# acids-ircam/RAVE

Measured on NVIDIA H100. Metric: audio-seconds/s (v2 train step fwd+bwd, 48 kHz), higher is better.
Workload: dtype bf16

## Files before the change

include/rave_b200.h:

```cpp
#ifndef RAVE_B200_H
#define RAVE_B200_H

#include <stddef.h>
#include <stdint.h>

#ifdef __cplusplus
extern "C" {
#endif

#define RAVE_ACT_NONE 0
#define RAVE_ACT_LEAKY 1
#define RAVE_ACT_SNAKE 2

#define RAVE_PREC_FP32 0
#define RAVE_PREC_BF16 1
#define RAVE_PREC_TF32 2

int rave_b200_version(void);
const char *rave_b200_last_error(void);
unsigned long long rave_b200_launch_count(void);

int rave_pqmf_analysis_fwd(const float *x, const float *taps, float *y, int B, int T, int Lout,
                           int ntaps, int pad_l, int flip_sign, void *stream);
int rave_pqmf_synthesis_fwd(const float *x, const float *w, float *out, int B, int L, int K,
// ... 65 lines not shown
                           void *stream);
int rave_time_stack_nhwc(const float *x, void *out_bf16, int B, int C, int T, int F, long sb, long st, int Fp, int Cp, int kt,
                         int pt, void *stream);
int rave_time_stack_nhwc_bwd(const void *g_bf16, float *gx, int B, int C, int T, int F, int Fp, int Cp, int kt, int pt,
                             void *stream);
int rave_time_stack_nhwc_dil(const float *x, void *out_bf16, int B, int C, int T, int F, long sb, long st, int Fp, int Cp,
                             int kt, int pt, int dil, void *stream);
int rave_time_stack_nhwc_dil_bwd(const void *g_bf16, float *gx, int B, int C, int T, int F, int Fp, int Cp, int kt, int pt,
                                 int dil, void *stream);
int rave_l1_stats_f32(const float *t, const float *v, float *stats, long n, void *stream);
int rave_l1_grad_f32(const float *t, const float *v, const float *d, float *gt, float *gv, long n, void *stream);
int rave_leaky_fm_fwd(const float *x, float *a, float *stats, long H, float slope, void *stream);
int rave_leaky_fm_bwd(const float *a, const float *g, const float *d, float *gx, long H, float slope, void *stream);
int rave_leaky_fm_stack_fwd(const float *x, float *a, float *stats, void *xs_bf16, long Rh, int T, int F, int C, int Fp,
                            float slope, void *stream);
int rave_leaky_fm_stack_bwd(const float *a, const void *gxs_bf16, const float *ga, const float *d, float *gx, long Rh, int T,
                            int F, int C, int Fp, float slope, void *stream);
int rave_leaky_fm_stack_dil_fwd(const float *x, float *a, float *stats, void *xs_bf16, long Rh, int T, int F, int C, int Fp,
                                int dil, float slope, void *stream);
int rave_leaky_fm_stack_dil_bwd(const float *a, const void *gxs_bf16, const float *ga, const float *d, float *gx, long Rh,
                                int T, int F, int C, int Fp, int dil, float slope, void *stream);
int rave_snake_cl_fwd(const void *h_bf16, const float *alpha, void *a_bf16, long rows, int C, void *stream);
int rave_snake_cl_bwd(const void *ga_bf16, const void *h_bf16, const float *alpha, const void *add_bf16, void *gh_bf16,
                      float *dalpha, long rows, int C, void *stream);
int rave_conv1d_tc_wgrad(const void *P_bf16, const void *Q_bf16, float *dwt, float *dbias, int B, int Cm, int Lp,
                         int p_pitch, int Cn, int Lq, int q_pitch, int K, int stride, int dil, int pad_l,
                         void *stream);
int rave_tapmajor_to_weight_f32(const float *dwt, float *dw, int Cm, int Cn, int K, int transpose, int splits,
                                void *stream);
int rave_conv1d_c1_fwd(const float *x, const float *w, const float *bias, float *out_f32, void *out_act_bf16,
                       int R, int x_pitch, int Lin, int Cout, int Lout, int out_pitch, int K, int stride,
                       int pad_l, int act, float slope, void *stream);
int rave_conv1d_c1_wgrad_splits(int R, int Lout);
int rave_conv1d_c1_wgrad(const void *g_bf16, const float *x, float *dwt, int R, int x_pitch, int Lin, int Cout,
                         int Cg, int Lout, int g_pitch, int K, int stride, int pad_l, void *stream);
int rave_conv1d_c1_dgrad(const void *g_bf16, const float *w, float *dx, int R, int x_pitch, int Lin, int Cout,
                         int Cg, int Lout, int g_pitch, int K, int stride, int pad_l, void *stream);
int rave_colsum_bf16(const void *g_bf16, float *out, int R, int L, int pitch, int Cg, int C, void *stream);
int rave_im2col_c1(const float *src, void *X_bf16, int R, int src_pitch, int src_len, int Lin, int Lout,
                   int out_pitch, int K, int stride, int pad_l, int period, int pool, void *stream);
int rave_gather_c1(const float *P, float *dsrc, int R, int src_pitch, int src_len, int Lin, int Lout, int p_pitch,
                   int K, int stride, int pad_l, int period, int pool, void *stream);
int rave_im2col_cin(const float *src, void *X_bf16, int R, int cin, int src_pitch, int src_len, int Lin, int Lout,
                    int out_pitch, int W, int K, int stride, int pad_l, int period, int pool, void *stream);
int rave_gather_cin(const float *P, float *dsrc, int R, int cin, int src_pitch, int src_len, int Lin, int Lout,
                    int p_pitch, int W, int K, int stride, int pad_l, int period, int pool, void *stream);
int rave_fm_stats(const void *a_bf16, float *stats, int Bh, int L, int pitch, int C, float slope, void *stream);
int rave_fm_grad(const void *a_bf16, const float *dstats, void *gout_bf16, int Bh, int L, int pitch, int C,
                 float slope, void *stream);
int rave_score_stats(const float *score, float *stats, int Bh, int L, int pitch, int C, void *stream);
int rave_score_grad(const float *score, const float *dstats, void *gout_bf16, int Bh, int L, int pitch, int C,
                    void *stream);

int rave_spectral_stats(const void *X_c64, const void *Y_c64, float *stats, long n, float eps, void *stream);
int rave_spectral_grad(const void *X_c64, const void *Y_c64, void *dY_c64, const float *stats, const float *gup,
                       long n, float eps, void *stream);
int rave_stft_frames(const float *x, const float *window, float *frames, int N, int T, int n_fft, int hop,
                     void *stream);
int rave_stft_frames_bwd(const float *dframes, const float *window, float *dx, int N, int T, int n_fft, int hop,
                         void *stream);
int rave_stft_frames_valid(const float *x, const float *window, float *frames, int N, int T, int n_fft, int hop,
                           float scale, void *stream);
int rave_stft_frames_valid_bwd(const float *dframes, const float *window, float *dx, int N, int T, int n_fft, int hop,
                               float scale, void *stream);
int rave_rfft_bwd_scale(const void *G_c64, void *Z_c64, long N, int F, int bins, long sN, long sF, long sB,
                        void *stream);

int rave_weight_prep_tc(const float *v, const float *g, float *norm, void *outA_bf16, const int *tapsA, int nA,
                        void *outB_bf16, const int *tapsB, int nB, int C0, int C1, int K, int C0p, int C1p,
                        void *stream);
int rave_weight_norm_bwd_tapmajor(const float *dwt, const float *v, const float *g, const float *norm, float *dv,
                                  float *dg, int C0, int C1, int K, int C0p, int C1p, int splits, void *stream);
typedef struct rave_wprep_layer {
  const float *v, *g;
  float *norm;
  void *outA, *outB;
  const float *dwt;
  float *dv, *dg;
  int C0, C1, K, C0p, C1p, nA, nB, splits;
  int tapsA[32], tapsB[32];
} rave_wprep_layer;
int rave_weight_prep_tc_multi(int n, const rave_wprep_layer *layers, void *stream);
int rave_weight_prep_tc_multi_x3(int n, const rave_wprep_layer *layers, void *stream);
int rave_weight_norm_bwd_multi(int n, const rave_wprep_layer *layers, void *stream);
int rave_ncl_to_cl(const float *x, void *y_bf16, float *y_f32, int B, int C, int L, int act, float slope,
                   const float *alpha, void *stream);
int rave_cl_to_ncl(const float *x_cl, float *y, int B, int C, int L, void *stream);
int rave_ncl_to_cl_x3(const float *x, void *y_bf16, int B, int C, int L, void *stream);
int rave_act_to_bf16(const float *x, void *y_bf16, int B, int C, int L, int act, float slope,
                     const float *alpha, void *stream);
int rave_weight_to_tapmajor_bf16(const float *w, void *wt_bf16, int Cout, int Cin, int K, int transpose,
                                 int flip, void *stream);

int rave_noise_fir_fwd(const float *h, const float *M, const float *noise, float *out, int B, int C, int NB, int T,
                       int TS, void *stream);
int rave_noise_fir_bwd(const float *h, const float *M, const float *noise, const float *dout, float *dh, int B, int C,
                       int NB, int T, int TS, void *stream);

int rave_mel_log1p_fwd(const void *X_c64, const int *band, const float *weights, float *out, int N, int F, int bins,
                       int M, int nnz, float scale, void *stream);
int rave_mel_log1p_bwd(const void *X_c64, const int *band, const float *weights, const float *dy, void *dX_c64, int N,
                       int F, int bins, int M, int nnz, float scale, void *stream);

int rave_gru_fwd(const float *gi, const float *w_hh, const float *b_hh, float *h_out, float *save, int B, int T, int H,
                 void *stream);
int rave_gru_bwd(const float *dy, const float *save, const float *w_hh, float *dgi, float *dgh, int B, int T, int H,
                 void *stream);
int rave_gemm_f32_splits(int M, int N, int K);
int rave_gemm_f32(const float *A, long sam, long sak, const float *B, long sbk, long sbn, const float *bias, float *C,
// ... 25 lines not shown
```

rave_b200/_lib.py:

```python
import ctypes
import os
from ctypes import c_float, c_int, c_long, c_size_t, c_ulonglong, c_void_p, c_char_p

_HERE = os.path.dirname(os.path.abspath(__file__))
LIB_PATH = os.path.join(_HERE, "csrc", "librave_b200.so")

_P, _I, _F, _L = c_void_p, c_int, c_float, c_long

SIGNATURES = {
    "rave_b200_version": (c_int, []),
    "rave_b200_last_error": (c_char_p, []),
    "rave_b200_launch_count": (c_ulonglong, []),
    "rave_pqmf_analysis_fwd": (c_int, [_P, _P, _P, _I, _I, _I, _I, _I, _I, _P]),
    "rave_pqmf_synthesis_fwd": (c_int, [_P, _P, _P, _I, _I, _I, _I, _F, _I, _P]),
    "rave_pqmf_analysis_fast": (c_int, [_P, _P, _P, _P, _I, _I, _I, _I, _I, _P]),
    "rave_pqmf_synthesis_fast": (c_int, [_P, _P, _P, _P, _I, _I, _I, _F, _I, _P]),
    "rave_conv1d_gather_f32": (c_int, [_P, _P, _P, _P, _P, _I, _I, _I, _I, _I, _I, _I, _I, _I, _L, _L,
                                       _I, _F, _P, _I, _F, _P, _P, _P]),
    "rave_conv1d_scatter_f32": (c_int, [_P, _P, _P, _P, _P, _I, _I, _I, _I, _I, _I, _I, _I, _I, _L, _L,
                                        _I, _F, _P, _I, _F, _P, _P, _P]),
    "rave_conv1d_wgrad_workspace_bytes": (c_size_t, [_I, _I, _I, _I, _I]),
    "rave_conv1d_wgrad_f32": (c_int, [_P, _P, _P, _I, _I, _I, _I, _I, _I, _I, _I, _I, _L, _L, _I, _I,
                                      _F, _P, _P, _P]),
    "rave_weight_norm_fwd": (c_int, [_P, _P, _P, _P, _I, _I, _P]),
# ... 5 lines not shown
    "rave_reparam_fwd": (c_int, [_P, _P, _P, _P, _I, _I, _I, _P]),
    "rave_mmd_fwd": (c_int, [_P, _P, _P, _P, _I, _I, _I, _P]),
    "rave_mmd_bwd": (c_int, [_P, _P, _P, _P, _I, _I, _I, _P]),
    "rave_sphere_norm_fwd": (c_int, [_P, _P, _P, _I, _I, _I, _P]),
    "rave_sphere_norm_bwd": (c_int, [_P, _P, _P, _P, _I, _I, _I, _P]),
    "rave_latent_moments": (c_int, [_P, _I, _I, _I, _I, _P, _P, _P]),
    "rave_latent_moments_workspace_bytes": (c_long, [_I, _I, _I]),
    "rave_conv1d_tc_supported": (c_int, [_I, _I, _I, _I, _I]),
    "rave_dilated_unit_tc_supported": (c_int, [_I, _I]),
    "rave_dilated_unit_tc_fwd": (c_int, [_P, _P, _P, _P, _P, _P, _I, _I, _I, _I, _I, _I, _F, _F, _I, _F, _P]),
    "rave_conv1d_tc_plan": (c_int, [_I, _I, _I, _I, _I]),
    "rave_conv1d_tc_pp_stages": (c_int, [_I, _I, _I, _I, _I, _I, _I]),
    "rave_conv1d_tc_pp_fwd_stages": (c_int, [_I, _I, _I, _I, _I]),
    "rave_conv1d_tc_fwd": (c_int, [_P, _P, _P, _P, _P, _P, _P, _F, _P, _P, _I, _I, _I, _I, _I, _I, _I, _I, _I, _I, _I,
                                   _F, _I, _I, _I, _P, _I, _P]),
    "rave_conv1d_tc_fwd_x3": (c_int, [_P, _P, _P, _P, _P, _F, _P, _P, _I, _I, _I, _I, _I, _I, _I, _I, _I, _I, _I, _F, _I,
                                      _I, _I, _I, _P]),
    "rave_weight_prep_tc_multi_x3": (c_int, [_I, _P, _P]),
    "rave_ncl_to_cl_x3": (c_int, [_P, _P, _I, _I, _I, _P]),
    "rave_conv1d_tc_wgrad": (c_int, [_P, _P, _P, _P, _I, _I, _I, _I, _I, _I, _I, _I, _I, _I, _I, _P]),
    "rave_tapmajor_to_weight_f32": (c_int, [_P, _P, _I, _I, _I, _I, _I, _P]),
    "rave_conv1d_tc_wgrad_splits": (c_int, [_I, _I, _I, _I, _I]),
    "rave_time_stack_cl": (c_int, [_P, _P, _I, _I, _I, _I, _I, _I, _I, _I, _P]),
    "rave_time_stack_cl_bwd": (c_int, [_P, _P, _I, _I, _I, _I, _I, _I, _I, _I, _P]),
    "rave_time_stack_nhwc": (c_int, [_P, _P, _I, _I, _I, _I, ctypes.c_long, ctypes.c_long, _I, _I, _I, _I, _P]),
    "rave_time_stack_nhwc_bwd": (c_int, [_P, _P, _I, _I, _I, _I, _I, _I, _I, _I, _P]),
    "rave_time_stack_nhwc_dil": (c_int, [_P, _P, _I, _I, _I, _I, ctypes.c_long, ctypes.c_long, _I, _I, _I, _I, _I, _P]),
    "rave_time_stack_nhwc_dil_bwd": (c_int, [_P, _P, _I, _I, _I, _I, _I, _I, _I, _I, _I, _P]),
    "rave_l1_stats_f32": (c_int, [_P, _P, _P, ctypes.c_long, _P]),
    "rave_leaky_fm_fwd": (c_int, [_P, _P, _P, ctypes.c_long, ctypes.c_float, _P]),
    "rave_leaky_fm_bwd": (c_int, [_P, _P, _P, _P, ctypes.c_long, ctypes.c_float, _P]),
    "rave_leaky_fm_stack_fwd": (c_int, [_P, _P, _P, _P, ctypes.c_long, _I, _I, _I, _I, ctypes.c_float, _P]),
    "rave_leaky_fm_stack_bwd": (c_int, [_P, _P, _P, _P, _P, ctypes.c_long, _I, _I, _I, _I, ctypes.c_float, _P]),
    "rave_leaky_fm_stack_dil_fwd": (c_int, [_P, _P, _P, _P, ctypes.c_long, _I, _I, _I, _I, _I, ctypes.c_float, _P]),
    "rave_leaky_fm_stack_dil_bwd": (c_int, [_P, _P, _P, _P, _P, ctypes.c_long, _I, _I, _I, _I, _I, ctypes.c_float, _P]),
    "rave_l1_grad_f32": (c_int, [_P, _P, _P, _P, _P, ctypes.c_long, _P]),
    "rave_snake_cl_fwd": (c_int, [_P, _P, _P, ctypes.c_long, _I, _P]),
    "rave_snake_cl_bwd": (c_int, [_P, _P, _P, _P, _P, _P, ctypes.c_long, _I, _P]),
    "rave_weight_prep_tc": (c_int, [_P, _P, _P, _P, _P, _I, _P, _P, _I, _I, _I, _I, _I, _I, _P]),
    "rave_weight_norm_bwd_tapmajor": (c_int, [_P, _P, _P, _P, _P, _P, _I, _I, _I, _I, _I, _I, _P]),
    "rave_conv1d_c1_fwd": (c_int, [_P, _P, _P, _P, _P, _I, _I, _I, _I, _I, _I, _I, _I, _I, _I, _F, _P]),
    "rave_conv1d_c1_wgrad_splits": (c_int, [_I, _I]),
    "rave_conv1d_c1_wgrad": (c_int, [_P, _P, _P, _I, _I, _I, _I, _I, _I, _I, _I, _I, _I, _P]),
    "rave_conv1d_c1_dgrad": (c_int, [_P, _P, _P, _I, _I, _I, _I, _I, _I, _I, _I, _I, _I, _P]),
    "rave_colsum_bf16": (c_int, [_P, _P, _I, _I, _I, _I, _I, _P]),
    "rave_im2col_c1": (c_int, [_P, _P, _I, _I, _I, _I, _I, _I, _I, _I, _I, _I, _I, _P]),
    "rave_gather_c1": (c_int, [_P, _P, _I, _I, _I, _I, _I, _I, _I, _I, _I, _I, _I, _P]),
    "rave_im2col_cin": (c_int, [_P, _P, _I, _I, _I, _I, _I, _I, _I, _I, _I, _I, _I, _I, _I, _P]),
    "rave_gather_cin": (c_int, [_P, _P, _I, _I, _I, _I, _I, _I, _I, _I, _I, _I, _I, _I, _I, _P]),
    "rave_fm_stats": (c_int, [_P, _P, _I, _I, _I, _I, _F, _P]),
    "rave_fm_grad": (c_int, [_P, _P, _P, _I, _I, _I, _I, _F, _P]),
    "rave_score_stats": (c_int, [_P, _P, _I, _I, _I, _I, _P]),
    "rave_score_grad": (c_int, [_P, _P, _P, _I, _I, _I, _I, _P]),
    "rave_spectral_stats": (c_int, [_P, _P, _P, _L, _F, _P]),
    "rave_spectral_grad": (c_int, [_P, _P, _P, _P, _P, _L, _F, _P]),
    "rave_stft_frames": (c_int, [_P, _P, _P, _I, _I, _I, _I, _P]),
    "rave_stft_frames_bwd": (c_int, [_P, _P, _P, _I, _I, _I, _I, _P]),
    "rave_stft_frames_valid": (c_int, [_P, _P, _P, _I, _I, _I, _I, _F, _P]),
    "rave_stft_frames_valid_bwd": (c_int, [_P, _P, _P, _I, _I, _I, _I, _F, _P]),
    "rave_rfft_bwd_scale": (c_int, [_P, _P, _L, _I, _I, _L, _L, _L, _P]),
    "rave_mel_log1p_fwd": (c_int, [_P, _P, _P, _P, _I, _I, _I, _I, _I, _F, _P]),
    "rave_mel_log1p_bwd": (c_int, [_P, _P, _P, _P, _P, _I, _I, _I, _I, _I, _F, _P]),
    "rave_gru_fwd": (c_int, [_P, _P, _P, _P, _P, _I, _I, _I, _P]),
    "rave_gru_bwd": (c_int, [_P, _P, _P, _P, _P, _I, _I, _I, _P]),
    "rave_gemm_f32_splits": (c_int, [_I, _I, _I]),
    "rave_gemm_f32": (c_int, [_P, _L, _L, _P, _L, _L, _P, _P, _L, _P, _I, _I, _I, _P, _I, _P]),
    "rave_noise_fir_fwd": (c_int, [_P, _P, _P, _P, _I, _I, _I, _I, _I, _P]),
    "rave_noise_fir_bwd": (c_int, [_P, _P, _P, _P, _P, _I, _I, _I, _I, _I, _P]),
    "rave_adam_multi": (c_int, [_I, _P, _P, _P, _P, _P, _P, _P, _F, _F, _F, _P]),
    "rave_weight_prep_tc_multi": (c_int, [_I, _P, _P]),
    "rave_weight_norm_bwd_multi": (c_int, [_I, _P, _P]),
    "rave_ncl_to_cl": (c_int, [_P, _P, _P, _I, _I, _I, _I, _F, _P, _P]),
    "rave_cl_to_ncl": (c_int, [_P, _P, _I, _I, _I, _P]),
    "rave_act_to_bf16": (c_int, [_P, _P, _I, _I, _I, _I, _F, _P, _P]),
    "rave_weight_to_tapmajor_bf16": (c_int, [_P, _P, _I, _I, _I, _I, _I, _P]),
    "rave_prior_latent_classes": (c_int, [_P, _P, _P, _P, _P, _I, _I, _I, _I, _I, _P]),
    "rave_prior_embed_fwd": (c_int, [_P, _P, _P, _P, _P, _I, _I, _I, _I, _I, _I, _I, _F, _P]),
    "rave_prior_embed_wgrad": (c_int, [_P, _P, _P, _P, _P, _I, _I, _I, _I, _I, _I, _I, _F, _P]),
    "rave_gate_fwd": (c_int, [_P, _P, _I, _I, _I, _I, _P]),
    "rave_gate_bwd": (c_int, [_P, _P, _P, _I, _I, _I, _I, _P]),
    "rave_prior_head_ce_fwd": (c_int, [_P, _P, _P, _P, _P, _I, _I, _I, _I, _I, _I, _F, _P]),
    "rave_prior_head_ce_bwd": (c_int, [_P, _P, _P, _P, _P, _P, _P, _P, _I, _I, _I, _I, _I, _I, _F, _P]),
}



class WPrepLayer(ctypes.Structure):
    _fields_ = [("v", c_void_p), ("g", c_void_p), ("norm", c_void_p), ("outA", c_void_p), ("outB", c_void_p),
                ("dwt", c_void_p), ("dv", c_void_p), ("dg", c_void_p),
                ("C0", c_int), ("C1", c_int), ("K", c_int), ("C0p", c_int), ("C1p", c_int), ("nA", c_int),
                ("nB", c_int), ("splits", c_int), ("tapsA", c_int * 32), ("tapsB", c_int * 32)]


_lib = None


class RaveB200Error(RuntimeError):
    pass


def load():
    global _lib
    if _lib is not None:
        return _lib
    if not os.path.isfile(LIB_PATH):
        raise RaveB200Error(
            f"{LIB_PATH} not found: build it with `python -c 'import __graft_entry__ as g; g.build()'` "
            "(rave_b200 has no CPU or PyTorch fallback)")
# ... 55 lines not shown
```

rave_b200/core.py:

```python
from typing import Callable, Optional, Sequence

import numpy as np
import torch
import torch.nn as nn


def mod_sigmoid(x):
    return 2 * torch.sigmoid(x) ** 2.3 + 1e-7


def get_augmented_latent_size(latent_size: int, noise_augmentation: int):
    return latent_size + noise_augmentation


def hinge_gan(score_real, score_fake):
    loss_dis = (torch.relu(1 - score_real) + torch.relu(1 + score_fake)).mean()
    loss_gen = -score_fake.mean()
    return loss_dis, loss_gen


def ls_gan(score_real, score_fake):
    loss_dis = ((score_real - 1).pow(2) + score_fake.pow(2)).mean()
    loss_gen = (score_fake - 1).pow(2).mean()
    return loss_dis, loss_gen
# ... 154 lines not shown
        f = fb.detach().cpu()
        rows, wts, off = [], [], 0
        for m in range(f.shape[1]):
            nz = torch.nonzero(f[:, m]).reshape(-1)
            lo, hi = (int(nz[0]), int(nz[-1]) + 1) if nz.numel() else (0, 0)
            rows.append((lo, hi, off))
            wts.append(f[lo:hi, m])
            off += hi - lo
        w = torch.cat(wts) if off else torch.zeros(1)
        table = (torch.tensor(rows, dtype=torch.int32).to(fb.device), w.contiguous().to(fb.device))
        self.__dict__["_bands"] = (fb, fb._version, table)
        return table

    def encode_log1p(self, x: torch.Tensor) -> torch.Tensor:
        from . import ops
        batch, channels, T = x.shape
        w = self.spectrogram.window
        if x.requires_grad and torch.is_grad_enabled():
            X = ops.rfft(ops.stft_frames(x.reshape(-1, T), w, self.n_fft, self.hop_length), self._rfft_bw())
            band, wts = self.band_table()
            return ops.MelLog1pFn.apply(X, band, wts, self.n_mels, 1.0 / float(self._win_energy()), batch, channels)
        with torch.no_grad():
            frames = ops.stft_frames(x.detach().reshape(-1, T), w, self.n_fft, self.hop_length)
            X = torch.fft.rfft(frames)
            band, wts = self.band_table()
            return ops.mel_log1p(X, band, wts, self.n_mels, 1.0 / float(self._win_energy()), batch, channels)

    def _rfft_bw(self):
        w = self.spectrogram.window
        hit = self.__dict__.get("_rfft_bw_cache")
        if hit is None or hit.device != w.device:
            bw = torch.full((self.n_fft // 2 + 1,), 0.5 * self.n_fft)
            bw[0] = bw[-1] = self.n_fft
            hit = self.__dict__["_rfft_bw_cache"] = bw.to(w.device)
        return hit

    def _win_energy(self):
        w = self.spectrogram.window
        hit = self.__dict__.get("_energy")
        if hit is None or hit[0] is not w or hit[1] != w._version:
            hit = self.__dict__["_energy"] = (w, w._version, float(w.detach().double().square().sum().cpu()))
        return hit[2]


class AudioDistanceV1(nn.Module):

    def __init__(self, multiscale_stft: Callable[[], nn.Module], log_epsilon: float) -> None:
        super().__init__()
        self.multiscale_stft = multiscale_stft()
        self.log_epsilon = log_epsilon

    def forward(self, x, y):
        mstft = self.multiscale_stft
        if (x.is_cuda and not x.requires_grad and isinstance(mstft, MultiScaleSTFT) and mstft.magnitude
                and x.dtype == torch.float32):
            from . import ops
            distance = 0.
            for sx, sy in zip(mstft.complex_stfts(x), mstft.complex_stfts(y)):
                distance = distance + ops.spectral_distance(sx, sy, self.log_epsilon)
            return {"spectral_distance": distance}
        stfts_x = self.multiscale_stft(x)
        stfts_y = self.multiscale_stft(y)
        distance = 0.
        for sx, sy in zip(stfts_x, stfts_y):
            logx = torch.log(sx + self.log_epsilon)
            logy = torch.log(sy + self.log_epsilon)
            distance = distance + mean_difference(sx, sy, norm="L2", relative=True) \
                + mean_difference(logx, logy, norm="L1")
        return {"spectral_distance": distance}


def _is_recurrent(module) -> bool:
    return hasattr(module, "gru_state") or hasattr(module, "temporal")


@torch.enable_grad()
def get_rave_receptive_field(model, n_channels=1):
    from . import engine, pqmf
    N = 2 ** 15
    device = next(iter(model.parameters())).device
    was_training, precision = model.training, engine.precision()
    recurrent = [m for m in model.modules() if _is_recurrent(m)]
    banks = [m for m in model.modules() if isinstance(m, pqmf.PQMF)]
    model.eval()
    engine.set_precision("fp32")
    for m in recurrent:
        m.disable()
    for m in banks:
        m.exact_taps = True
    try:
        while True:
            x = torch.randn(1, model.n_channels, N, requires_grad=True, device=device)
            z = model.encode(x)
            z = model.encoder.reparametrize(z)[0]
            y = model.decode(z)
            (grad,) = torch.autograd.grad(y[0, 0, N // 2], x, allow_unused=True)
            if grad is None:
                raise RuntimeError("get_rave_receptive_field: the output does not depend on the input (an encoder "
                                   "that detaches its output, e.g. a VariationalEncoder in phase 2)")
            left_grad, right_grad = grad.reshape(-1).chunk(2, 0)
            if left_grad[0] == 0 and right_grad[-1] == 0:
                break
            N *= 2
        left_rf = int((left_grad != 0).sum())
        right_rf = int((right_grad != 0).sum())
    finally:
        for m in recurrent:
            m.enable()
        for m in banks:
            m.exact_taps = False
        engine.set_precision(precision)
        model.train(was_training)
# ... 39 lines not shown
```

rave_b200/csrc/api.cu:

```cuda
#include <stdarg.h>

#include <atomic>

#include "common.cuh"

namespace rave {
static thread_local char g_err[512] = "";
static std::atomic<unsigned long long> g_launches{0};

void set_error(const char *fmt, ...) {
  va_list ap;
  va_start(ap, fmt);
  vsnprintf(g_err, sizeof(g_err), fmt, ap);
  va_end(ap);
}
void count_launch(int n) { g_launches.fetch_add((unsigned long long)n, std::memory_order_relaxed); }
}

extern "C" int rave_b200_version(void) { return 105; }
extern "C" const char *rave_b200_last_error(void) { return rave::g_err; }
extern "C" unsigned long long rave_b200_launch_count(void) {
  return rave::g_launches.load(std::memory_order_relaxed);
}
```

rave_b200/csrc/spectral.cu:

```cuda
#include "common.cuh"

namespace rave {

__global__ void __launch_bounds__(256)
spectral_stats_kernel(const float2 *__restrict__ X, const float2 *__restrict__ Y, float *__restrict__ stats, long n,
                      float eps, const BlockSum bs) {
  __shared__ float red[3][8];
  float s0 = 0.f, s1 = 0.f, s2 = 0.f;
  for (long i = blockIdx.x * 256L + threadIdx.x; i < n; i += (long)gridDim.x * 256) {
    const float2 x = X[i], y = Y[i];
    const float ax = sqrtf(x.x * x.x + x.y * x.y);
    const float ay = sqrtf(y.x * y.x + y.y * y.y);
    const float d = ax - ay;
    s0 = fmaf(d, d, s0);
    s1 = fmaf(ax, ax, s1);
    s2 += fabsf(logf(ax + eps) - logf(ay + eps));
  }
#pragma unroll
  for (int o = 16; o > 0; o >>= 1) {
    s0 += __shfl_xor_sync(0xffffffffu, s0, o);
    s1 += __shfl_xor_sync(0xffffffffu, s1, o);
    s2 += __shfl_xor_sync(0xffffffffu, s2, o);
  }
  const int wid = threadIdx.x >> 5, lane = threadIdx.x & 31;
  if (lane == 0) { red[0][wid] = s0; red[1][wid] = s1; red[2][wid] = s2; }
  __syncthreads();
  if (threadIdx.x < 3) {
    float t = 0.f;
    for (int i = 0; i < 8; ++i) t += red[threadIdx.x][i];
    block_sum_put(bs, threadIdx.x, t);
  }
  if (block_sum_finish(bs, stats) && threadIdx.x == 0) stats[4] = stats[0] / stats[1] + stats[2] / (float)n;
}

__global__ void __launch_bounds__(256)
spectral_grad_kernel(const float2 *__restrict__ X, const float2 *__restrict__ Y, float2 *__restrict__ dY,
                     const float *__restrict__ stats, const float *__restrict__ gup, long n, float eps) {
  const float g = gup[0];
  const float c_lin = g / stats[1], c_log = g / (float)n;
  for (long i = blockIdx.x * 256L + threadIdx.x; i < n; i += (long)gridDim.x * 256) {
    const float2 x = X[i], y = Y[i];
    const float ax = sqrtf(x.x * x.x + x.y * x.y);
    const float ay = sqrtf(y.x * y.x + y.y * y.y);
    const float dl = logf(ax + eps) - logf(ay + eps);
    const float sg = dl > 0.f ? 1.f : (dl < 0.f ? -1.f : 0.f);
    const float dmag = c_lin * (-2.f) * (ax - ay) - c_log * sg / (ay + eps);
    const float inv = ay > 0.f ? dmag / ay : 0.f;
    dY[i] = make_float2(y.x * inv, y.y * inv);
  }
}

__global__ void __launch_bounds__(256)
stft_frames_kernel(const float *__restrict__ x, const float *__restrict__ w, float *__restrict__ frames, long total4,
                   int T, int n_fft, int hop, int F, int vec_ok) {
  const int h = n_fft >> 1;
  const int q = n_fft >> 2;
  const int qs = 31 - __clz(q);
  for (long i = blockIdx.x * 256L + threadIdx.x; i < total4; i += (long)gridDim.x * 256) {
    const int t = (int)(i & (q - 1)) << 2;
    const long nf = i >> qs;
    const int f = (int)(nf % F);
    const long n = nf / F;
    const int j0 = f * hop + t - h;
    const float4 ww = __ldg(reinterpret_cast<const float4 *>(w + t));
    const float *xn = x + n * T;
    float4 xv;
    if (vec_ok && j0 >= 0 && j0 + 3 < T) {
      xv = __ldg(reinterpret_cast<const float4 *>(xn + j0));
    } else {
      float e[4];
#pragma unroll
      for (int u = 0; u < 4; ++u) {
        int j = j0 + u;
        if (j < 0) j = -j;
        if (j >= T) j = 2 * (T - 1) - j;
        e[u] = __ldg(xn + j);
      }
      xv = make_float4(e[0], e[1], e[2], e[3]);
    }
    reinterpret_cast<float4 *>(frames)[i] = make_float4(ww.x * xv.x, ww.y * xv.y, ww.z * xv.z, ww.w * xv.w);
  }
}

__device__ __forceinline__ float stft_ola_at(const float *__restrict__ d, const float *__restrict__ w, int p, int n_fft,
                                             int hop, int F) {
  float acc = 0.f;
  int f_hi = p / hop;
  if (f_hi > F - 1) f_hi = F - 1;
  int f_lo = (p - n_fft + hop) / hop;
  if (p - n_fft + 1 <= 0) f_lo = 0;
  for (int f = f_lo; f <= f_hi; ++f) {
    const int t = p - f * hop;
    acc = fmaf(__ldg(w + t), __ldg(d + (size_t)f * n_fft + t), acc);
  }
  return acc;
}

__global__ void __launch_bounds__(256)
stft_frames_bwd_kernel(const float *__restrict__ dframes, const float *__restrict__ w, float *__restrict__ dx, long total,
                       int T, int n_fft, int hop, int F) {
  const int h = n_fft >> 1;
// ... 78 lines not shown
  long blocks = (total4 + 255) / 256;
  if (blocks > 132 * 16) blocks = 132 * 16;
  const int vec_ok = (T % 4 == 0) && (((uintptr_t)x & 15) == 0);
  stft_frames_kernel<<<(int)blocks, 256, 0, (cudaStream_t)stream>>>(x, window, frames, total4, T, n_fft, hop, F, vec_ok);
  RAVE_CHECK_LAUNCH("stft_frames");
  return 0;
}

extern "C" int rave_stft_frames_bwd(const float *dframes, const float *window, float *dx, int N, int T, int n_fft,
                                    int hop, void *stream) {
  using namespace rave;
  RAVE_CHECK_ARG(dframes && window && dx && N > 0 && T > n_fft / 2 && n_fft >= 2 && hop > 0 && n_fft % hop == 0,
                 "stft_frames_bwd: bad argument");
  const int F = 1 + T / hop;
  const long total = (long)N * T;
  long blocks = (total + 255) / 256;
  if (blocks > 132 * 16) blocks = 132 * 16;
  stft_frames_bwd_kernel<<<(int)blocks, 256, 0, (cudaStream_t)stream>>>(dframes, window, dx, total, T, n_fft, hop, F);
  RAVE_CHECK_LAUNCH("stft_frames_bwd");
  return 0;
}

extern "C" int rave_stft_frames_valid(const float *x, const float *window, float *frames, int N, int T, int n_fft, int hop,
                                      float scale, void *stream) {
  using namespace rave;
  RAVE_CHECK_ARG(x && window && frames && N > 0 && T >= n_fft && n_fft >= 16 && (n_fft & (n_fft - 1)) == 0 && hop > 0,
                 "stft_frames_valid: bad argument (T >= n_fft, n_fft a power of two >= 16)");
  const int F = 1 + (T - n_fft) / hop;
  const long total4 = (long)N * F * (n_fft / 4);
  long blocks = (total4 + 255) / 256;
  if (blocks > 132 * 16) blocks = 132 * 16;
  const int vec_ok = (T % 4 == 0) && (hop % 4 == 0) && (((uintptr_t)x & 15) == 0);
  stft_frames_valid_kernel<<<(int)blocks, 256, 0, (cudaStream_t)stream>>>(x, window, frames, total4, T, n_fft, hop, F,
                                                                          scale, vec_ok);
  RAVE_CHECK_LAUNCH("stft_frames_valid");
  return 0;
}

extern "C" int rave_stft_frames_valid_bwd(const float *dframes, const float *window, float *dx, int N, int T, int n_fft,
                                          int hop, float scale, void *stream) {
  using namespace rave;
  RAVE_CHECK_ARG(dframes && window && dx && N > 0 && T >= n_fft && n_fft >= 16 && hop > 0,
                 "stft_frames_valid_bwd: bad argument");
  const int F = 1 + (T - n_fft) / hop;
  const long total = (long)N * T;
  long blocks = (total + 255) / 256;
  if (blocks > 132 * 16) blocks = 132 * 16;
  stft_frames_valid_bwd_kernel<<<(int)blocks, 256, 0, (cudaStream_t)stream>>>(dframes, window, dx, total, T, n_fft, hop,
                                                                              F, scale);
  RAVE_CHECK_LAUNCH("stft_frames_valid_bwd");
  return 0;
}

extern "C" int rave_spectral_stats(const void *X, const void *Y, float *stats, long n, float eps, void *stream) {
  using namespace rave;
  RAVE_CHECK_ARG(X && Y && stats && n > 0, "spectral_stats: bad argument");
  long blocks = (n + 255) / 256;
  if (blocks > 132 * 8) blocks = 132 * 8;
  BlockSum bs;
  if (int rc = block_sum_begin(&bs, blocks, 3, (cudaStream_t)stream)) return rc;
  spectral_stats_kernel<<<(int)blocks, 256, 0, (cudaStream_t)stream>>>((const float2 *)X, (const float2 *)Y, stats, n,
                                                                       eps, bs);
  block_sum_end(bs, (cudaStream_t)stream);
  RAVE_CHECK_LAUNCH("spectral_stats");
  return 0;
}

extern "C" int rave_spectral_grad(const void *X, const void *Y, void *dY, const float *stats, const float *gup, long n,
                                  float eps, void *stream) {
  using namespace rave;
  RAVE_CHECK_ARG(X && Y && dY && stats && gup && n > 0, "spectral_grad: bad argument");
  long blocks = (n + 255) / 256;
  if (blocks > 132 * 16) blocks = 132 * 16;
  spectral_grad_kernel<<<(int)blocks, 256, 0, (cudaStream_t)stream>>>((const float2 *)X, (const float2 *)Y,
                                                                      (float2 *)dY, stats, gup, n, eps);
  RAVE_CHECK_LAUNCH("spectral_grad");
  return 0;
}

namespace rave {

constexpr int MEL_FT = 8;

__global__ void __launch_bounds__(256)
mel_log1p_kernel(const float2 *__restrict__ X, const int *__restrict__ band, const float *__restrict__ wts,
                 float *__restrict__ out, int F, int bins, int M, int nnz, float scale) {
  extern __shared__ float sm[];
  float *P = sm;
  float *W = P + MEL_FT * bins;
  int *bd = reinterpret_cast<int *>(W + nnz);
  const int n = blockIdx.y, f0 = blockIdx.x * MEL_FT;
  const int Fo = F - 1;
  const int nf = min(MEL_FT, Fo - f0);
  const float2 *Xn = X + ((size_t)n * F + f0) * bins;
  for (int i = threadIdx.x; i < nf * bins; i += blockDim.x) {
    const float2 v = Xn[i];
    P[i] = fmaf(v.x, v.x, v.y * v.y);
  }
  for (int i = threadIdx.x; i < nnz; i += blockDim.x) W[i] = wts[i];
  for (int i = threadIdx.x; i < 3 * M; i += blockDim.x) bd[i] = band[i];
  __syncthreads();
  for (int o = threadIdx.x; o < M * MEL_FT; o += blockDim.x) {
    const int m = o / MEL_FT, f = o % MEL_FT;
    if (f >= nf) continue;
    const int lo = bd[3 * m], hi = bd[3 * m + 1], off = bd[3 * m + 2];
    const float *p = P + f * bins;
    float acc = 0.f;
    for (int k = lo; k < hi; ++k) acc = fmaf(W[off + k - lo], p[k], acc);
    out[((size_t)n * M + m) * Fo + f0 + f] = log1pf(scale * acc);
  }
}

__global__ void __launch_bounds__(256)
mel_log1p_bwd_kernel(const float2 *__restrict__ X, const int *__restrict__ band, const float *__restrict__ wts,
                     const float *__restrict__ dy, float2 *__restrict__ dX, int F, int bins, int M, int nnz, float scale) {
  extern __shared__ float sm[];
  float *P = sm;
  float *W = P + MEL_FT * bins;
  float *G = W + nnz;
  int *bd = reinterpret_cast<int *>(G + M * MEL_FT);
  const int n = blockIdx.y, f0 = blockIdx.x * MEL_FT;
  const int Fo = F - 1;
  const int nf = min(MEL_FT, F - f0);
  const int nv = min(MEL_FT, Fo - f0);
  const float2 *Xn = X + ((size_t)n * F + f0) * bins;
  float2 *dXn = dX + ((size_t)n * F + f0) * bins;
  for (int i = threadIdx.x; i < nf * bins; i += blockDim.x) {
    const float2 v = Xn[i];
// ... 173 lines not shown
```

rave_b200/model.py:

```python
import math
from typing import Callable, Dict, Iterable, Optional

import contextlib

import torch
import torch.nn as nn

from . import blocks, core

_default_loss_weights = {
    "audio_distance": 1.,
    "multiband_audio_distance": 1.,
    "adversarial": 1.,
    "feature_matching": 20,
}


def _pqmf_encode(pqmf, x: torch.Tensor):
    batch_size = x.shape[:-2]
    x_multiband = x.reshape(-1, 1, x.shape[-1])
    x_multiband = pqmf(x_multiband)
    return x_multiband.reshape(*batch_size, -1, x_multiband.shape[-1])


# ... 193 lines not shown
        feature_real, feature_fake = [], []
        for scale in features:
            true, fake = zip(*map(lambda x: torch.split(x, x.shape[0] // 2, 0), scale))
            feature_real.append(true)
            feature_fake.append(fake)
        return feature_real, feature_fake

    def compute_losses(self, x_raw, is_dis_step: bool, eps: Optional[torch.Tensor] = None):
        batch_size = x_raw.shape[:-2]
        if getattr(self, "_static_enc_prep", False) and not self.warmed_up:
            from . import engine
            engine.disable_static_prep(self.encoder)
            self._static_enc_prep = False
        self.encoder.set_warmed_up(self.warmed_up)
        self.decoder.set_warmed_up(self.warmed_up)

        z, x_multiband = self.encode(x_raw, return_mb=True)
        if eps is not None:
            z, reg = self.encoder.reparametrize(z, eps)[:2]
        else:
            z, reg = self.encoder.reparametrize(z)[:2]

        y = self.decoder(z)
        if self.output_mode == "pqmf":
            y_multiband = y
            y_raw = _pqmf_decode(self.pqmf, y, batch_size=batch_size, n_channels=self.n_channels)
        else:
            y_raw = y
            y_multiband = _pqmf_encode(self.pqmf, y)
        y_raw = y_raw[..., :x_raw.shape[-1]]
        y_multiband = y_multiband[..., :x_multiband.shape[-1]]

        if self.valid_signal_crop:
            left_rf, right_rf = self._receptive_field_host()
            if left_rf + right_rf:
                dim = x_multiband.shape[1]
                x_multiband = x_multiband[..., left_rf // dim:]
                y_multiband = y_multiband[..., left_rf // dim:]
                if right_rf:
                    x_multiband = x_multiband[..., :-right_rf // dim]
                    y_multiband = y_multiband[..., :-right_rf // dim]

        from . import discriminator
        side = None
        if y_raw.is_cuda and self.warmed_up and discriminator.DISC_STREAMS > 1:
            if getattr(self, "_loss_stream", None) is None:
                self._loss_stream = torch.cuda.Stream()
            side = self._loss_stream
            cur = torch.cuda.current_stream()
            side.wait_stream(cur)
            for t in (x_multiband, y_multiband, x_raw, y_raw):
                t.record_stream(side)
        distances = {}
        with torch.cuda.stream(side) if side is not None else contextlib.nullcontext():
            for k, v in self.multiband_audio_distance(x_multiband, y_multiband).items():
                distances[f"multiband_{k}"] = self.weights["multiband_audio_distance"] * v
            for k, v in self.audio_distance(x_raw, y_raw).items():
                distances[f"fullband_{k}"] = self.weights["audio_distance"] * v

        feature_matching_distance = 0.
        fused = None
        if self.warmed_up:
            y_d = y_raw.detach() if is_dis_step else y_raw
            xy = torch.cat([x_raw, y_d], 0)
            fused = self._fused_feature_matching(xy, fake_grad_only=not is_dis_step)
        if fused is not None:
            feature_matching_distance, loss_dis, loss_adv, pred_real, pred_fake = fused
        elif self.warmed_up:
            from . import engine
            with engine.fake_rows_only(not is_dis_step):
                features = self.discriminator(xy)
            feature_real, feature_fake = self.split_features(features)
            loss_dis = 0
            loss_adv = 0
            pred_real = 0
            pred_fake = 0
            kw = getattr(self.feature_matching_fun, "keywords", None)
            on_bases = (kw is not None and getattr(self.feature_matching_fun, "func", None) is core.mean_difference
                        and kw.get("norm", "L1") == "L1")
            skip = self.num_skipped_features
            tapped = []
            for scale, scale_real, scale_fake in zip(features, feature_real, feature_fake):
                terms = []
                n_terms = len(scale[skip:])
                for full, real, fake in zip(scale[skip:], scale_real[skip:], scale_fake[skip:]):
                    base = getattr(full, "_cl_base", None) if on_bases else None
                    st = getattr(full, "_fm_stats", None) if on_bases else None
                    if st is not None:
                        tapped.append((st, real.numel(), 1.0 / (n_terms * len(feature_real))))
                    elif base is not None:
                        terms.append(core.mean_difference_halves(base, real.numel(), bool(kw.get("relative", False))))
                    else:
                        terms.append(self.feature_matching_fun(real, fake))
                if terms:
                    feature_matching_distance = feature_matching_distance + sum(terms) / (n_terms * len(feature_real))
                _dis, _adv = self.gan_loss(scale_real[-1], scale_fake[-1])
                pred_real = pred_real + scale_real[-1].mean()
                pred_fake = pred_fake + scale_fake[-1].mean()
                loss_dis = loss_dis + _dis
                loss_adv = loss_adv + _adv
            if tapped:
                feature_matching_distance = feature_matching_distance + core.stacked_l1_terms(
                    tapped, bool(kw.get("relative", False)))
        else:
            pred_real = x_raw.new_zeros(())
            pred_fake = x_raw.new_zeros(())
            loss_dis = x_raw.new_zeros(())
# ... 157 lines not shown
```

rave_b200/ops.py:

```python
from typing import Optional, Tuple

import torch

from . import _lib
from ._lib import call, ptr, stream_ptr

ACT_NONE, ACT_LEAKY, ACT_SNAKE = 0, 1, 2


def _f32c(t: Optional[torch.Tensor]) -> Optional[torch.Tensor]:
    if t is None:
        return None
    if t.dtype != torch.float32:
        raise _lib.RaveB200Error(f"expected float32 tensor, got {t.dtype}")
    return t if t.is_contiguous() else t.contiguous()


def conv_out_len(Lin: int, K: int, stride: int, dil: int, pad_l: int, pad_r: int) -> int:
    return (Lin + pad_l + pad_r - dil * (K - 1) - 1) // stride + 1



def _gather(src, w, bias, res, out, K, stride, dil, pad_l, ws_m, ws_c, act, slope, alpha,
            post_act=0, post_slope=0.0, post_x=None, post_alpha=None):
# ... 828 lines not shown
def im2col_c1(src, Lin, Lout, out_pitch, K, stride, pad_l, period=1, pool=1):
    src = _f32c(src)
    Bs, T = src.shape
    R = Bs * period
    X = torch.empty(R, out_pitch, 16, dtype=torch.bfloat16, device=src.device)
    call("rave_im2col_c1", ptr(src), ptr(X), R, T, T, Lin, Lout, out_pitch, K, stride, pad_l, period, pool,
         stream_ptr())
    return X


def gather_c1(P_cl, src_shape, Lin, Lout, K, stride, pad_l, period=1, pool=1, batch0=0):
    P_cl = _f32c(P_cl)
    R, p_pitch, _ = P_cl.shape
    Bs, T = src_shape
    dsrc = torch.zeros(Bs, T, dtype=torch.float32, device=P_cl.device)
    if R != (Bs - batch0) * period:
        raise _lib.RaveB200Error("gather_c1: row count does not match the source batches")
    call("rave_gather_c1", ptr(P_cl), dsrc.data_ptr() + batch0 * T * 4, R, T, T, Lin, Lout, p_pitch, K, stride, pad_l,
         period, pool, stream_ptr())
    return dsrc


def cin_width(cin, K):
    return 16 if cin * K <= 16 else 32


def im2col_cin(src, Lin, Lout, out_pitch, K, stride, pad_l, period=1, pool=1):
    src = _f32c(src)
    Bs, cin, T = src.shape
    W = cin_width(cin, K)
    R = Bs * period
    X = torch.empty(R, out_pitch, W, dtype=torch.bfloat16, device=src.device)
    call("rave_im2col_cin", ptr(src), ptr(X), R, cin, T, T, Lin, Lout, out_pitch, W, K, stride, pad_l, period, pool,
         stream_ptr())
    return X


def gather_cin(P_cl, src_shape, Lin, Lout, K, stride, pad_l, period=1, pool=1, batch0=0):
    P_cl = _f32c(P_cl)
    R, p_pitch, W = P_cl.shape
    Bs, cin, T = src_shape
    dsrc = torch.zeros(Bs, cin, T, dtype=torch.float32, device=P_cl.device)
    if R != (Bs - batch0) * period or W != cin_width(cin, K):
        raise _lib.RaveB200Error("gather_cin: P does not match the source batches or the row width")
    call("rave_gather_cin", ptr(P_cl), dsrc.data_ptr() + batch0 * cin * T * 4, R, cin, T, T, Lin, Lout, p_pitch, W, K,
         stride, pad_l, period, pool, stream_ptr())
    return dsrc



class SpectralDistanceFn(torch.autograd.Function):

    @staticmethod
    def forward(ctx, X, Y, eps):
        if X.dtype != torch.complex64 or Y.dtype != torch.complex64 or X.shape != Y.shape:
            raise _lib.RaveB200Error("spectral distance expects two complex64 spectrograms of equal shape")
        if X.stride() == Y.stride() and X.transpose(-1, -2).is_contiguous():
            X, Y = X.transpose(-1, -2), Y.transpose(-1, -2)
            ctx.transposed = True
        else:
            X, Y = X.contiguous(), Y.contiguous()
            ctx.transposed = False
        n = X.numel()
        stats = torch.zeros(5, dtype=torch.float32, device=X.device)
        call("rave_spectral_stats", ptr(torch.view_as_real(X)), ptr(torch.view_as_real(Y)), ptr(stats), n,
             float(eps), stream_ptr())
        ctx.save_for_backward(X, Y)
        ctx.stats = stats
        ctx.eps = float(eps)
        return stats[4]

    @staticmethod
    def backward(ctx, g):
        X, Y = ctx.saved_tensors
        stats = ctx.stats
        n = X.numel()
        g = g.to(torch.float32)
        if g.dim() != 0 or not g.is_cuda:
            raise _lib.RaveB200Error("spectral distance: the upstream gradient must be a CUDA scalar")
        dY = torch.empty_like(Y, memory_format=torch.contiguous_format)
        call("rave_spectral_grad", ptr(torch.view_as_real(X)), ptr(torch.view_as_real(Y)),
             ptr(torch.view_as_real(dY)), stats.data_ptr(), g.data_ptr(), n, ctx.eps, stream_ptr())
        return None, (dY.transpose(-1, -2) if ctx.transposed else dY), None


def spectral_distance(X, Y, eps):
    return SpectralDistanceFn.apply(X, Y, eps)


class StftFramesFn(torch.autograd.Function):

    @staticmethod
    def forward(ctx, x, window, n_fft, hop):
        x = _f32c(x)
        N, T = x.shape
        F = 1 + T // hop
        frames = torch.empty(N, F, n_fft, dtype=torch.float32, device=x.device)
        call("rave_stft_frames", ptr(x), ptr(window), ptr(frames), N, T, n_fft, hop, stream_ptr())
        ctx.save_for_backward(window)
        ctx.dims = (N, T, n_fft, hop)
        return frames

    @staticmethod
    def backward(ctx, g):
        (window,) = ctx.saved_tensors
        N, T, n_fft, hop = ctx.dims
        g = _f32c(g)
        dx = torch.empty(N, T, dtype=torch.float32, device=g.device)
        call("rave_stft_frames_bwd", ptr(g), ptr(window), ptr(dx), N, T, n_fft, hop, stream_ptr())
        return dx, None, None, None


def stft_frames(x, window, n_fft, hop):
    return StftFramesFn.apply(x, window, n_fft, hop)


class StftFramesValidFn(torch.autograd.Function):

    @staticmethod
    def forward(ctx, x, window, n_fft, hop, scale):
        x = _f32c(x)
        N, T = x.shape
        F = 1 + (T - n_fft) // hop
        frames = torch.empty(N, F, n_fft, dtype=torch.float32, device=x.device)
        call("rave_stft_frames_valid", ptr(x), ptr(window), ptr(frames), N, T, n_fft, hop, float(scale), stream_ptr())
        ctx.save_for_backward(window)
        ctx.dims = (N, T, n_fft, hop, float(scale))
        return frames

    @staticmethod
    def backward(ctx, g):
        (window,) = ctx.saved_tensors
        N, T, n_fft, hop, scale = ctx.dims
        g = _f32c(g)
        dx = torch.empty(N, T, dtype=torch.float32, device=g.device)
        call("rave_stft_frames_valid_bwd", ptr(g), ptr(window), ptr(dx), N, T, n_fft, hop, scale, stream_ptr())
        return dx, None, None, None, None


def stft_frames_valid(x, window, n_fft, hop, scale):
# ... 314 lines not shown
```

Baseline: 2297.

## Fuse framing, FFT and spectral distance into one kernel for no-grad steps

Adds a custom shared-memory radix-4 FFT kernel that frames both signals with reflect padding and windowing, packs x and y as real and imaginary parts, and reduces the spectral-distance statistics in one pass without materialising spectrograms. It is used when no gradient is needed, and the discriminator step's distance computation now runs under no_grad so it takes this path. The grad path now builds frames with the custom framing op and uses rfft/irfft directly, folding the irfft-backward scaling into the grad kernel. This adds a hand-written FFT with its own numerical behaviour and a special case for discriminator steps.

```diff
diff --git a/include/rave_b200.h b/include/rave_b200.h
--- a/include/rave_b200.h
+++ b/include/rave_b200.h
@@ -141,9 +141,11 @@
 int rave_score_grad(const float *score, const float *dstats, void *gout_bf16, int Bh, int L, int pitch, int C,
                     void *stream);
 
+int rave_spectral_distance_fwd(const float *x, const float *y, const float *window, float *stats, int rows, int T,
+                               int n_fft, float eps, void *stream);
 int rave_spectral_stats(const void *X_c64, const void *Y_c64, float *stats, long n, float eps, void *stream);
-int rave_spectral_grad(const void *X_c64, const void *Y_c64, void *dY_c64, const float *stats, const float *gup,
-                       long n, float eps, void *stream);
+int rave_spectral_grad(const void *X_c64, const void *Y_c64, void *Z_c64, const float *stats, const float *gup,
+                       long n, int bins, float eps, void *stream);
 int rave_stft_frames(const float *x, const float *window, float *frames, int N, int T, int n_fft, int hop,
                      void *stream);
 int rave_stft_frames_bwd(const float *dframes, const float *window, float *dx, int N, int T, int n_fft, int hop,
diff --git a/rave_b200/_lib.py b/rave_b200/_lib.py
--- a/rave_b200/_lib.py
+++ b/rave_b200/_lib.py
@@ -81,8 +81,9 @@
     "rave_fm_grad": (c_int, [_P, _P, _P, _I, _I, _I, _I, _F, _P]),
     "rave_score_stats": (c_int, [_P, _P, _I, _I, _I, _I, _P]),
     "rave_score_grad": (c_int, [_P, _P, _P, _I, _I, _I, _I, _P]),
+    "rave_spectral_distance_fwd": (c_int, [_P, _P, _P, _P, _I, _I, _I, _F, _P]),
     "rave_spectral_stats": (c_int, [_P, _P, _P, _L, _F, _P]),
-    "rave_spectral_grad": (c_int, [_P, _P, _P, _P, _P, _L, _F, _P]),
+    "rave_spectral_grad": (c_int, [_P, _P, _P, _P, _P, _L, _I, _F, _P]),
     "rave_stft_frames": (c_int, [_P, _P, _P, _I, _I, _I, _I, _P]),
     "rave_stft_frames_bwd": (c_int, [_P, _P, _P, _I, _I, _I, _I, _P]),
     "rave_stft_frames_valid": (c_int, [_P, _P, _P, _I, _I, _I, _I, _F, _P]),
diff --git a/rave_b200/core.py b/rave_b200/core.py
--- a/rave_b200/core.py
+++ b/rave_b200/core.py
@@ -230,12 +230,24 @@
 
     def forward(self, x, y):
         mstft = self.multiscale_stft
+        if (x.is_cuda and not (y.requires_grad and torch.is_grad_enabled()) and isinstance(mstft, MultiScaleSTFT)
+                and mstft.magnitude and x.dtype == torch.float32 and y.dtype == torch.float32 and not mstft.normalized
+                and all(64 <= s <= 4096 and s & (s - 1) == 0 and x.shape[-1] > s // 2 for s in mstft.scales)):
+            from . import ops
+            T = x.shape[-1]
+            windows = [getattr(mstft, f"window_{s}") for s in mstft.scales]
+            return {"spectral_distance": ops.spectral_distance_fwd(x.reshape(-1, T), y.reshape(-1, T), windows,
+                                                                   mstft.scales, self.log_epsilon)}
         if (x.is_cuda and not x.requires_grad and isinstance(mstft, MultiScaleSTFT) and mstft.magnitude
-                and x.dtype == torch.float32):
+                and x.dtype == torch.float32 and not mstft.normalized and all(x.shape[-1] > s // 2 for s in mstft.scales)):
             from . import ops
+            T = x.shape[-1]
+            x2, y2 = x.reshape(-1, T), y.reshape(-1, T)
             distance = 0.
-            for sx, sy in zip(mstft.complex_stfts(x), mstft.complex_stfts(y)):
-                distance = distance + ops.spectral_distance(sx, sy, self.log_epsilon)
+            for s in mstft.scales:
+                w = getattr(mstft, f"window_{s}")
+                distance = distance + ops.spectral_distance(ops.stft_frames(x2, w, s, s // 4),
+                                                            ops.stft_frames(y2, w, s, s // 4), self.log_epsilon)
             return {"spectral_distance": distance}
         stfts_x = self.multiscale_stft(x)
         stfts_y = self.multiscale_stft(y)
diff --git a/rave_b200/csrc/api.cu b/rave_b200/csrc/api.cu
--- a/rave_b200/csrc/api.cu
+++ b/rave_b200/csrc/api.cu
@@ -17,7 +17,7 @@
 void count_launch(int n) { g_launches.fetch_add((unsigned long long)n, std::memory_order_relaxed); }
 }
 
-extern "C" int rave_b200_version(void) { return 105; }
+extern "C" int rave_b200_version(void) { return 106; }
 extern "C" const char *rave_b200_last_error(void) { return rave::g_err; }
 extern "C" unsigned long long rave_b200_launch_count(void) {
   return rave::g_launches.load(std::memory_order_relaxed);
diff --git a/rave_b200/csrc/spectral.cu b/rave_b200/csrc/spectral.cu
--- a/rave_b200/csrc/spectral.cu
+++ b/rave_b200/csrc/spectral.cu
@@ -1,6 +1,125 @@
 #include "common.cuh"
 
 namespace rave {
+
+constexpr int FFT_PTS = 4096;
+constexpr int FFT_THREADS = 256;
+
+__device__ __forceinline__ float2 cmul(float2 a, float2 b) {
+  return make_float2(a.x * b.x - a.y * b.y, a.x * b.y + a.y * b.x);
+}
+__device__ __forceinline__ float2 cadd(float2 a, float2 b) { return make_float2(a.x + b.x, a.y + b.y); }
+__device__ __forceinline__ float2 csub(float2 a, float2 b) { return make_float2(a.x - b.x, a.y - b.y); }
+__device__ __forceinline__ int bitrev(int a, int logn) { return (int)(__brev((unsigned)a) >> (32 - logn)); }
+
+__device__ __forceinline__ void fft_twiddles(float2 *tw, int logn) {
+  const int n = 1 << logn;
+  for (int k = threadIdx.x; k < n / 2; k += blockDim.x) {
+    float sn, cs;
+    sincospif(2.f * (float)k / (float)n, &sn, &cs);
+    tw[k] = make_float2(cs, -sn);
+  }
+}
+
+__device__ void fft_dif(float2 *z, const float2 *tw, int logn) {
+  int lm = logn - 1;
+  for (; lm >= 1; lm -= 2) {
+    const int m = 1 << (lm - 1);
+    for (int b = threadIdx.x; b < FFT_PTS / 4; b += FFT_THREADS) {
+      const int j = b & (m - 1);
+      const int base = ((b >> (lm - 1)) << (lm + 1)) + j;
+      float2 a0 = z[base], a1 = z[base + m], a2 = z[base + 2 * m], a3 = z[base + 3 * m];
+      const float2 w4a = tw[j << (logn - 1 - lm)], w4b = tw[(j + m) << (logn - 1 - lm)];
+      const float2 w2 = tw[j << (logn - lm)];
+      const float2 b0 = cadd(a0, a2), b2 = cmul(csub(a0, a2), w4a);
+      const float2 b1 = cadd(a1, a3), b3 = cmul(csub(a1, a3), w4b);
+      z[base] = cadd(b0, b1);
+      z[base + m] = cmul(csub(b0, b1), w2);
+      z[base + 2 * m] = cadd(b2, b3);
+      z[base + 3 * m] = cmul(csub(b2, b3), w2);
+    }
+    __syncthreads();
+  }
+  if (lm == 0) {
+    for (int b = threadIdx.x; b < FFT_PTS / 2; b += FFT_THREADS) {
+      const float2 a = z[2 * b], c = z[2 * b + 1];
+      z[2 * b] = cadd(a, c);
+      z[2 * b + 1] = csub(a, c);
+    }
+    __syncthreads();
+  }
+}
+
+__device__ __forceinline__ int reflect_index(int i, int T) {
+  if (i < 0) i = -i;
+  if (i >= T) i = 2 * (T - 1) - i;
+  return i;
+}
+
+__device__ __forceinline__ void unpack_xy(float2 zk, float2 zm, float2 &X, float2 &Y) {
+  X = make_float2(0.5f * (zk.x + zm.x), 0.5f * (zk.y - zm.y));
+  Y = make_float2(0.5f * (zk.y + zm.y), 0.5f * (zm.x - zk.x));
+}
+
+__global__ void __launch_bounds__(FFT_THREADS)
+spectral_distance_fwd_kernel(const float *__restrict__ x, const float *__restrict__ y, const float *__restrict__ w,
+                             float *__restrict__ stats, int rows, int T, int logn, int F, float eps, const BlockSum bs) {
+  extern __shared__ float2 fsm[];
+  float2 *z = fsm, *tw = fsm + FFT_PTS;
+  const int n = 1 << logn, h = n >> 1, hop = n >> 2, G = FFT_PTS >> logn;
+  const long frames = (long)rows * F;
+  const long tiles = (frames + G - 1) / G;
+  fft_twiddles(tw, logn);
+  float s0 = 0.f, s1 = 0.f, s2 = 0.f;
+  for (long tile = blockIdx.x; tile < tiles; tile += gridDim.x) {
+    __syncthreads();
+    for (int p = threadIdx.x; p < FFT_PTS; p += FFT_THREADS) {
+      const int t = p & (n - 1);
+      const long fi = tile * G + (p >> logn);
+      float2 v = make_float2(0.f, 0.f);
+      if (fi < frames) {
+        const long r = fi / F;
+        const int f = (int)(fi - r * F);
+        const long j = r * T + reflect_index(f * hop + t - h, T);
+        const float wt = __ldg(w + t);
+        v = make_float2(wt * __ldg(x + j), wt * __ldg(y + j));
+      }
+      z[p] = v;
+    }
+    __syncthreads();
+    fft_dif(z, tw, logn);
+    for (int q = threadIdx.x; q < G * (h + 1); q += FFT_THREADS) {
+      const int gi = q / (h + 1), k = q - gi * (h + 1);
+      if (tile * G + gi >= frames) continue;
+      const float2 *zf = z + (gi << logn);
+      float2 X, Y;
+      unpack_xy(zf[bitrev(k, logn)], zf[bitrev((n - k) & (n - 1), logn)], X, Y);
+      const float ax = sqrtf(X.x * X.x + X.y * X.y);
+      const float ay = sqrtf(Y.x * Y.x + Y.y * Y.y);
+      const float d = ax - ay;
+      s0 = fmaf(d, d, s0);
+      s1 = fmaf(ax, ax, s1);
+      s2 += fabsf(logf(ax + eps) - logf(ay + eps));
+    }
+  }
+  __shared__ float red[3][FFT_THREADS / 32];
+#pragma unroll
+  for (int o = 16; o > 0; o >>= 1) {
+    s0 += __shfl_xor_sync(0xffffffffu, s0, o);
+    s1 += __shfl_xor_sync(0xffffffffu, s1, o);
+    s2 += __shfl_xor_sync(0xffffffffu, s2, o);
+  }
+  const int wid = threadIdx.x >> 5, lane = threadIdx.x & 31;
+  if (lane == 0) { red[0][wid] = s0; red[1][wid] = s1; red[2][wid] = s2; }
+  __syncthreads();
+  if (threadIdx.x < 3) {
+    float t = 0.f;
+    for (int i = 0; i < FFT_THREADS / 32; ++i) t += red[threadIdx.x][i];
+    block_sum_put(bs, threadIdx.x, t);
+  }
+  if (block_sum_finish(bs, stats) && threadIdx.x == 0)
+    stats[4] = stats[0] / stats[1] + stats[2] / (float)((double)frames * (h + 1));
+}
 
 __global__ void __launch_bounds__(256)
 spectral_stats_kernel(const float2 *__restrict__ X, const float2 *__restrict__ Y, float *__restrict__ stats, long n,
@@ -34,8 +153,9 @@
 }
 
 __global__ void __launch_bounds__(256)
-spectral_grad_kernel(const float2 *__restrict__ X, const float2 *__restrict__ Y, float2 *__restrict__ dY,
-                     const float *__restrict__ stats, const float *__restrict__ gup, long n, float eps) {
+spectral_grad_kernel(const float2 *__restrict__ X, const float2 *__restrict__ Y, float2 *__restrict__ Z,
+                     const float *__restrict__ stats, const float *__restrict__ gup, long n, int bins, float eps) {
+  const float n_fft = (float)(2 * (bins - 1));
   const float g = gup[0];
   const float c_lin = g / stats[1], c_log = g / (float)n;
   for (long i = blockIdx.x * 256L + threadIdx.x; i < n; i += (long)gridDim.x * 256) {
@@ -46,7 +166,11 @@
     const float sg = dl > 0.f ? 1.f : (dl < 0.f ? -1.f : 0.f);
     const float dmag = c_lin * (-2.f) * (ax - ay) - c_log * sg / (ay + eps);
     const float inv = ay > 0.f ? dmag / ay : 0.f;
-    dY[i] = make_float2(y.x * inv, y.y * inv);
+    const float2 dy = make_float2(y.x * inv, y.y * inv);
+    const int k = (int)(i % bins);
+    const bool edge = (k == 0) || (k == bins - 1);
+    const float sc = edge ? n_fft : 0.5f * n_fft;
+    Z[i] = make_float2(dy.x * sc, edge ? 0.f : dy.y * sc);
   }
 }
 
@@ -231,6 +355,31 @@
   return 0;
 }
 
+static int spectral_logn(int n_fft) {
+  int l = 0;
+  while ((1 << l) < n_fft) ++l;
+  return l;
+}
+
+extern "C" int rave_spectral_distance_fwd(const float *x, const float *y, const float *window, float *stats, int rows,
+                                          int T, int n_fft, float eps, void *stream) {
+  using namespace rave;
+  RAVE_CHECK_ARG(x && y && window && stats && rows > 0 && n_fft >= 64 && n_fft <= FFT_PTS &&
+                     (n_fft & (n_fft - 1)) == 0 && T > n_fft / 2,
+                 "spectral_distance_fwd: bad argument (n_fft a power of two in [64, %d], T > n_fft/2)", FFT_PTS);
+  const int logn = spectral_logn(n_fft), F = 1 + T / (n_fft / 4);
+  const long tiles = ((long)rows * F + (FFT_PTS / n_fft) - 1) / (FFT_PTS / n_fft);
+  const long blocks = tiles < 132 * 4 ? tiles : 132 * 4;
+  const size_t smem = (size_t)(FFT_PTS + n_fft / 2) * sizeof(float2);
+  BlockSum bs;
+  if (int rc = block_sum_begin(&bs, blocks, 3, (cudaStream_t)stream)) return rc;
+  spectral_distance_fwd_kernel<<<(int)blocks, FFT_THREADS, smem, (cudaStream_t)stream>>>(x, y, window, stats, rows, T,
+                                                                                          logn, F, eps, bs);
+  block_sum_end(bs, (cudaStream_t)stream);
+  RAVE_CHECK_LAUNCH("spectral_distance_fwd");
+  return 0;
+}
+
 extern "C" int rave_spectral_stats(const void *X, const void *Y, float *stats, long n, float eps, void *stream) {
   using namespace rave;
   RAVE_CHECK_ARG(X && Y && stats && n > 0, "spectral_stats: bad argument");
@@ -245,14 +394,14 @@
   return 0;
 }
 
-extern "C" int rave_spectral_grad(const void *X, const void *Y, void *dY, const float *stats, const float *gup, long n,
-                                  float eps, void *stream) {
-  using namespace rave;
-  RAVE_CHECK_ARG(X && Y && dY && stats && gup && n > 0, "spectral_grad: bad argument");
+extern "C" int rave_spectral_grad(const void *X, const void *Y, void *Z, const float *stats, const float *gup, long n,
+                                  int bins, float eps, void *stream) {
+  using namespace rave;
+  RAVE_CHECK_ARG(X && Y && Z && stats && gup && n > 0 && bins > 1 && n % bins == 0, "spectral_grad: bad argument");
   long blocks = (n + 255) / 256;
   if (blocks > 132 * 16) blocks = 132 * 16;
   spectral_grad_kernel<<<(int)blocks, 256, 0, (cudaStream_t)stream>>>((const float2 *)X, (const float2 *)Y,
-                                                                      (float2 *)dY, stats, gup, n, eps);
+                                                                      (float2 *)Z, stats, gup, n, bins, eps);
   RAVE_CHECK_LAUNCH("spectral_grad");
   return 0;
 }
diff --git a/rave_b200/model.py b/rave_b200/model.py
--- a/rave_b200/model.py
+++ b/rave_b200/model.py
@@ -269,7 +269,8 @@
             for t in (x_multiband, y_multiband, x_raw, y_raw):
                 t.record_stream(side)
         distances = {}
-        with torch.cuda.stream(side) if side is not None else contextlib.nullcontext():
+        with torch.cuda.stream(side) if side is not None else contextlib.nullcontext(), \
+                torch.no_grad() if is_dis_step else contextlib.nullcontext():
             for k, v in self.multiband_audio_distance(x_multiband, y_multiband).items():
                 distances[f"multiband_{k}"] = self.weights["multiband_audio_distance"] * v
             for k, v in self.audio_distance(x_raw, y_raw).items():
diff --git a/rave_b200/ops.py b/rave_b200/ops.py
--- a/rave_b200/ops.py
+++ b/rave_b200/ops.py
@@ -904,15 +904,10 @@
 class SpectralDistanceFn(torch.autograd.Function):
 
     @staticmethod
-    def forward(ctx, X, Y, eps):
-        if X.dtype != torch.complex64 or Y.dtype != torch.complex64 or X.shape != Y.shape:
-            raise _lib.RaveB200Error("spectral distance expects two complex64 spectrograms of equal shape")
-        if X.stride() == Y.stride() and X.transpose(-1, -2).is_contiguous():
-            X, Y = X.transpose(-1, -2), Y.transpose(-1, -2)
-            ctx.transposed = True
-        else:
-            X, Y = X.contiguous(), Y.contiguous()
-            ctx.transposed = False
+    def forward(ctx, fx, fy, eps):
+        if fx.dtype != torch.float32 or fy.dtype != torch.float32 or fx.shape != fy.shape or fx.dim() != 3:
+            raise _lib.RaveB200Error("spectral distance expects two float32 [N, F, n_fft] frame tensors of equal shape")
+        X, Y = torch.fft.rfft(fx), torch.fft.rfft(fy)
         n = X.numel()
         stats = torch.zeros(5, dtype=torch.float32, device=X.device)
         call("rave_spectral_stats", ptr(torch.view_as_real(X)), ptr(torch.view_as_real(Y)), ptr(stats), n,
@@ -920,6 +915,7 @@
         ctx.save_for_backward(X, Y)
         ctx.stats = stats
         ctx.eps = float(eps)
+        ctx.n_fft = fx.shape[-1]
         return stats[4]
 
     @staticmethod
@@ -930,14 +926,25 @@
         g = g.to(torch.float32)
         if g.dim() != 0 or not g.is_cuda:
             raise _lib.RaveB200Error("spectral distance: the upstream gradient must be a CUDA scalar")
-        dY = torch.empty_like(Y, memory_format=torch.contiguous_format)
+        Z = torch.empty_like(Y)
         call("rave_spectral_grad", ptr(torch.view_as_real(X)), ptr(torch.view_as_real(Y)),
-             ptr(torch.view_as_real(dY)), stats.data_ptr(), g.data_ptr(), n, ctx.eps, stream_ptr())
-        return None, (dY.transpose(-1, -2) if ctx.transposed else dY), None
-
-
-def spectral_distance(X, Y, eps):
-    return SpectralDistanceFn.apply(X, Y, eps)
+             ptr(torch.view_as_real(Z)), stats.data_ptr(), g.data_ptr(), n, Y.shape[-1], ctx.eps, stream_ptr())
+        return None, torch.fft.irfft(Z, n=ctx.n_fft), None
+
+
+def spectral_distance(fx, fy, eps):
+    return SpectralDistanceFn.apply(fx, fy, eps)
+
+
+def spectral_distance_fwd(x, y, windows, scales, eps):
+    x, y = _f32c(x), _f32c(y)
+    if x.dim() != 2 or x.shape != y.shape:
+        raise _lib.RaveB200Error("spectral distance expects two [N, T] signals of equal shape")
+    N, T = x.shape
+    stats = torch.zeros(len(scales), 5, dtype=torch.float32, device=x.device)
+    for i, (w, n) in enumerate(zip(windows, scales)):
+        call("rave_spectral_distance_fwd", ptr(x), ptr(y), ptr(w), ptr(stats[i]), N, T, n, float(eps), stream_ptr())
+    return stats[:, 4].sum()
 
 
 class StftFramesFn(torch.autograd.Function):
```

Measured after the change: 2375 (median of 6 runs). +3.4%, better.
